# gotzmann/booster

Measured on AMD Instinct MI355X. Metric: decode tokens/sec Llama-3-8B Q4_K_M, higher is better.
Workload: dtype int8xint4/6 dot -> f32 (Q4_K/Q6_K weights x Q8_K activations), f16 KV; 1 GPU; Llama-3-8B Q4_K_M shapes (synthetic GGUF, random K-quant blocks), greedy batch-1 decode on 1xMI355X, 128-token prompt, n_ctx 2304, n_kv 133..2087; parallelism=single GPU, aql_runs=2, replay=AQL packets, fence scope NONE, own HSA queue (csrc/bamd_aql.h)

## Files before the change

### booster_amd/__init__.py

```python
import ctypes as C
import os

import numpy as np

_HERE = os.path.dirname(os.path.abspath(__file__))
LIB_PATH = os.environ.get("BAMD_LIB") or os.path.join(_HERE, "lib", "libbooster_amd.so")
_lib = None

F32, F16, Q4_K, Q5_K, Q6_K = 0, 1, 12, 13, 14


class BamdError(RuntimeError):
    pass


def lib():
    global _lib
    if _lib is None:
        if not os.path.exists(LIB_PATH):
            raise BamdError("libbooster_amd.so is not built (python -m booster_amd.build); there is no CPU fallback")
        try:
            import torch
        except ImportError:
            pass
        L = C.CDLL(LIB_PATH)
        vp, ci, cf, i64 = C.c_void_p, C.c_int, C.c_float, C.c_int64
        L.bamd_last_error.restype = C.c_char_p
        L.bamd_model_load.restype = vp; L.bamd_model_load.argtypes = [C.c_char_p, ci, ci, ci, ci, ci]
        L.bamd_model_free.argtypes = [vp]
        for n in ("bamd_model_n_vocab", "bamd_model_n_embd", "bamd_model_n_layer", "bamd_model_n_ctx_train"):
            getattr(L, n).argtypes = [vp]
        L.bamd_model_weight_bytes.restype = i64; L.bamd_model_weight_bytes.argtypes = [vp]
        L.bamd_model_tensor_raw.restype = i64; L.bamd_model_tensor_raw.argtypes = [vp, C.c_char_p, vp, i64]
        L.bamd_context_new.restype = vp; L.bamd_context_new.argtypes = [vp, ci]
        L.bamd_context_free.argtypes = [vp]
        L.bamd_n_ctx.argtypes = [vp]
        L.bamd_kv_cache_clear.argtypes = [vp]
        L.bamd_decode.argtypes = [vp, vp, ci, ci]
        L.bamd_get_logits.restype = C.POINTER(C.c_float); L.bamd_get_logits.argtypes = [vp]
        L.bamd_generate_greedy.argtypes = [vp, ci, ci, vp, C.POINTER(C.c_float)]
        L.bamd_kv_seq_rm.argtypes = [vp, ci, ci]; L.bamd_kv_seq_add.argtypes = [vp, ci, ci, ci]; L.bamd_kv_seq_div.argtypes = [vp, ci, ci, ci]
        L.bamd_stage_step.argtypes = [vp, C.c_int32, vp, ci, vp, vp, ci, ci, vp]
        L.bamd_stage_token_to.argtypes = [vp, vp, vp]
        L.bamd_stage_prefill.argtypes = [vp, vp, ci, ci, vp, vp, ci, vp]
        L.bamd_stage_argmax.argtypes = [vp, vp, C.POINTER(C.c_int32)]
        L.bamd_profile_step.argtypes = [vp, ci, vp, vp, vp]; L.bamd_profile_step_kinds.argtypes = [vp, ci, vp, vp, vp]
        L.bamd_timeline_step.argtypes = [vp, ci, ci, vp, ci, C.POINTER(ci)]
        L.bamd_set_prefill_batch.argtypes = [ci]; L.bamd_set_prefill_batch.restype = None
        L.bamd_bench_matvec.argtypes = [ci, ci, ci, ci, ci, ci, ci, C.POINTER(C.c_float)]
        L.bamd_op_quantize_q8_K.argtypes = [vp, i64, vp, cf, vp]
        L.bamd_op_mul_mat_vec.argtypes = [ci, vp, ci, ci, vp, vp, cf, vp, vp, ci]
        L.bamd_op_mul_mat_vec_argmax.argtypes = [ci, vp, ci, ci, vp, vp, cf, vp, ci, C.POINTER(C.c_int32)]
        L.bamd_op_ffn_gate_up.argtypes = [ci, vp, vp, ci, ci, vp, vp, cf, vp]
        L.bamd_op_mul_mat_batch.argtypes = [ci, vp, ci, ci, vp, ci, vp, cf, vp, vp, ci]
        L.bamd_op_get_row.argtypes = [ci, vp, ci, ci, ci, vp]
        L.bamd_op_attention.argtypes = [vp, vp, vp, vp, vp, vp, ci, ci, ci, ci, ci, ci, vp, vp]
        L.bamd_op_attention_batch.argtypes = [vp, vp, vp, vp, vp, vp, ci, ci, ci, ci, ci, ci, ci, ci, vp]
        L.bamd_op_rope_row.argtypes = [ci, ci, cf, cf, vp, vp]
        L.bamd_set_aql.argtypes = [ci]; L.bamd_set_aql.restype = None
        L.bamd_aql_runs.argtypes = [vp]
        _lib = L
    return _lib


def _chk(rc):
    if rc != 0:
        raise BamdError(lib().bamd_last_error().decode())


def _p(a):
    return None if a is None else a.ctypes.data_as(C.c_void_p)


def set_prefill_batch(on):
    lib().bamd_set_prefill_batch(int(on))


def set_aql(on):
    lib().bamd_set_aql(int(bool(on)))


def device_count():
    return lib().bamd_device_count()


class Model:

    def __init__(self, path, device=0, layer_first=0, layer_last=-1, with_embd=True, with_output=True):
        self.h = lib().bamd_model_load(os.fsencode(path), device, layer_first, layer_last, int(with_embd), int(with_output))
# ... 157 lines not shown

def op_ffn_gate_up(ttype, wg_raw, wu_raw, nrows, k, x, norm_w=None, eps=0.0):
    wg_raw = np.ascontiguousarray(wg_raw, np.uint8); wu_raw = np.ascontiguousarray(wu_raw, np.uint8)
    x = np.ascontiguousarray(x, np.float32)
    nw = None if norm_w is None else np.ascontiguousarray(norm_w, np.float32)
    y = np.zeros(nrows, np.float32)
    _chk(lib().bamd_op_ffn_gate_up(ttype, _p(wg_raw), _p(wu_raw), nrows, k, _p(x), _p(nw), eps, _p(y)))
    return y


def op_get_row(ttype, w_raw, nrows, k, row):
    w_raw = np.ascontiguousarray(w_raw, np.uint8)
    y = np.zeros(k, np.float32)
    _chk(lib().bamd_op_get_row(ttype, _p(w_raw), nrows, k, row, _p(y)))
    return y


def op_rope_row(pos, n_dims, freq_base, freq_scale=1.0, freq_factors=None):
    row = np.zeros(n_dims, np.float32)
    ff = None if freq_factors is None else np.ascontiguousarray(freq_factors, np.float32)
    _chk(lib().bamd_op_rope_row(pos, n_dims, freq_base, freq_scale, _p(ff), _p(row)))
    return row


def op_attention(q, k, v, k_cache, v_cache_t, rope_row, H, Hkv, hd, n_ctx, pos, prefill_mode=False, want_probs=False, long_path=False):
    q = np.ascontiguousarray(q, np.float32); k = np.ascontiguousarray(k, np.float32); v = np.ascontiguousarray(v, np.float32)
    rope_row = np.ascontiguousarray(rope_row, np.float32)
    assert k_cache.dtype == np.uint16 and v_cache_t.dtype == np.uint16 and k_cache.flags.c_contiguous and v_cache_t.flags.c_contiguous
    out = np.zeros(H * hd, np.float32)
    probs = np.zeros(n_ctx, np.float32) if want_probs else None
    _chk(lib().bamd_op_attention(_p(q), _p(k), _p(v), _p(k_cache), _p(v_cache_t), _p(rope_row), H, Hkv, hd, n_ctx, pos, int(prefill_mode) | (2 if (long_path or want_probs) else 0),
                                 _p(out), _p(probs)))
    return (out, probs) if want_probs else out


def op_attention_batch(q, k, v, k_cache, v_cache_t, rope, H, Hkv, hd, n_ctx, pos0, impl=0, ld=0):
    q = np.ascontiguousarray(q, np.float32).reshape(-1, H * hd)
    T = q.shape[0]
    k = np.ascontiguousarray(k, np.float32).reshape(T, Hkv * hd); v = np.ascontiguousarray(v, np.float32).reshape(T, Hkv * hd)
    rope = np.ascontiguousarray(rope, np.float32).reshape(n_ctx, hd)
    assert k_cache.dtype == np.uint16 and v_cache_t.dtype == np.uint16 and k_cache.flags.c_contiguous and v_cache_t.flags.c_contiguous
    assert k_cache.size == n_ctx * Hkv * hd and v_cache_t.size == n_ctx * Hkv * hd
    out = np.zeros((T, H * hd), np.float32)
    _chk(lib().bamd_op_attention_batch(_p(q), _p(k), _p(v), _p(k_cache), _p(v_cache_t), _p(rope), H, Hkv, hd, n_ctx, pos0, T, impl, ld, _p(out)))
    return out
```

### booster_amd/csrc/bamd_attention.hip

```cpp
#include "bamd_device.h"

#define BAMD_QK_NT 4
template <int GQ, int LG, bool SH, int NT = BAMD_QK_NT>
__global__ void __launch_bounds__(512) attn_qk_kernel(bamd_attn_args a) {
    constexpr int hd = 64 * LG, L = 8 * LG, hp = hd / 2;
    constexpr int NPAIR = (GQ + 1) * hp, IT = (NPAIR + 511) / 512;
    __shared__ __attribute__((aligned(16))) float qt[GQ * 256];
    __shared__ __attribute__((aligned(16))) unsigned short q16t[GQ * 256];
    __shared__ __attribute__((aligned(16))) unsigned short k16t[256];
    __shared__ __attribute__((aligned(16))) float scs[NT][GQ][64];
    const bamd_step_state * st = a.st;
    const int Hkv = a.Hkv, Ekv = Hkv * hd, n_ctx = a.n_ctx;
    const int hk = blockIdx.x, by = (int) blockIdx.y, gy = (int) gridDim.y;
    const int tid = threadIdx.x, lane = tid & 63, wave = wave_id(), e = lane & 7, r = lane >> 3;
    float2 xin[IT], cs[IT];
#pragma unroll
    for (int it = 0; it < IT; ++it) {
        const int idx = tid + it * 512, idc = idx < NPAIR ? idx : 0, hh = idc / hp, p = idc - hh * hp;
        const float * src = hh < GQ ? a.q + (size_t) (hk * GQ + hh) * hd : a.k + (size_t) hk * hd;
        xin[it] = ik_ld2f(src + 2 * p);
        cs[it] = ik_ld2f(a.rope_cur + 2 * p);
    }
    const float vst = ik_ld(a.v + hk * hd + (tid < hd ? tid : 0));
    const int pos = ik_ld(&st->pos), n_kv = ik_ld(&st->n_kv), cell = SH ? ik_ld(&st->cell) : pos;
// ... 36 lines not shown
#pragma unroll
            for (int g = 0; g < GQ; ++g) sc[g] = -INFINITY;
            bool live = i <= pos;
            if (SH) live = i < n_kv && (i == cell || (uint32_t) ik_ld(a.cellpos + (i < n_kv ? i : 0)) <= (uint32_t) pos);
            if (live) {
                uint4 kreg[4];
#pragma unroll
                for (int g = 0; g < 4; ++g) {
                    kreg[g] = make_uint4(0, 0, 0, 0);
                    if (g < LG) { const uint4 own = *(const uint4 *) (k16t + g * BAMD_KGRP + e * 8); kreg[g] = i == cell ? own : kpre[j][g < LG ? g : 0]; }
                }
#pragma unroll
                for (int g = 0; g < GQ; ++g) {
                    if (BAMD_QK_KNOCK & 2) { sc[g] = __uint_as_float(kreg[0].x ^ kreg[1 < LG ? 1 : 0].w) + qt[g * hd + e * 8]; continue; }
                    const float v = a.prefill_mode ? kq_chain<true>(kreg, L, nullptr, q16t + g * hd + e * 8) : kq_chain<false>(kreg, L, qt + g * hd + e * 8, nullptr);
                    sc[g] = a.prefill_mode ? hsum8_vecdot(v) : hsum8_tinyblas(v);
                }
            }
            if (e == 0) {
#pragma unroll
                for (int g = 0; g < GQ; ++g) scs[j][g][r * 8 + wave] = sc[g];
            }
        }
        __syncthreads();
        for (int q4 = tid; q4 < NT * GQ * 16; q4 += 512) {
            const int j = q4 / (GQ * 16), g = (q4 >> 4) % GQ, c4 = q4 & 15, tile = tile0 + j * gy;
            if (tile < tiles && (!(BAMD_QK_KNOCK & 4) || scs[j][g][c4 * 4] == 12345.f)) ik_st128f(rs, (uint32_t) ((hk * GQ + g) * n_ctx + tile * 64 + c4 * 4) * 4u, *(const float4 *) &scs[j][g][c4 * 4]);
        }
        if (tile0 + NT * gy < tiles) { __syncthreads(); BAMD_QK_PREFETCH(tile0 + NT * gy); }
    }
#undef BAMD_QK_PREFETCH
}

__device__ __forceinline__ double seq_expsum8_vt(const float * v, int n) {
    double sq = 0.0;
    for (int i = 0; i < n; i += 8) {
        const float * q = v + (i & ~63) + ((i & 63) >> 3);
        const float a0 = q[0] + q[32], a1 = q[8] + q[40], a2 = q[16] + q[48], a3 = q[24] + q[56];
        const float b0 = a0 + a2, b1 = a1 + a3;
        sq += (double) (b0 + b1);
    }
    return sq;
}
#define BAMD_SM_R 8
__global__ void __launch_bounds__(1024) attn_softmax_kernel(bamd_attn_args a) {
    __shared__ float redf[16];
    __shared__ double redd[16];
    const bamd_step_state * st = a.st;
    const int n_kv = st->n_kv, n_ctx = a.n_ctx;
    const int h = blockIdx.x;
    float * s = a.scores + (size_t) h * n_ctx;
    float * pr = a.probs + (size_t) h * n_ctx;
    const float scale = a.kq_scale;
    const int tid = threadIdx.x, lane = tid & 63, wave = wave_id(), nw = blockDim.x >> 6;
    const bool cached = n_kv <= BAMD_SM_R * (int) blockDim.x;
    float v[BAMD_SM_R];
    float mx = -INFINITY;
    if (cached) {
#pragma unroll
        for (int k = 0; k < BAMD_SM_R; ++k) { const int i = tid + k * blockDim.x; v[k] = i < n_kv ? s[vperm(i)] * scale : -INFINITY; mx = v[k] > mx ? v[k] : mx; }
    } else for (int i = tid; i < n_kv; i += blockDim.x) { const float w = s[vperm(i)] * scale; mx = w > mx ? w : mx; }
    for (int o = 32; o; o >>= 1) { const float om = __shfl_xor(mx, o); mx = om > mx ? om : mx; }
    if (lane == 0) redf[wave] = mx;
    __syncthreads();
    mx = redf[0]; for (int w = 1; w < nw; ++w) mx = redf[w] > mx ? redf[w] : mx;
    double sum = 0.0;
    if (cached) {
#pragma unroll
        for (int k = 0; k < BAMD_SM_R; ++k) {
            const int i = tid + k * blockDim.x;
            if (i < n_kv) {
                const float val = v_expf(v[k] - mx);
                v[k] = val;
                const float c = hsum8_tinyblas(val);
                if ((lane & 7) == 0) sum += (double) c;
            }
// ... 478 lines not shown
```

### booster_amd/csrc/bamd_attn_fused.h

```cpp
#pragma once
#include "bamd_device.h"

#define BAMD_ATTN_LDS_MAX (144 * 1024)
struct AttnEnvWG {
    int tid, wave, nthr;
    __device__ __forceinline__ AttnEnvWG() : tid((int) threadIdx.x), wave(wave_id()), nthr((int) blockDim.x) { }
    __device__ __forceinline__ void sync() const { __syncthreads(); }
    __device__ __forceinline__ float2 qk2(const bamd_attn_args & a, int role, int h, int hk, int hd, int rp) const {
        const float * rsrc = role == 1 ? a.k + (size_t) hk * hd : a.q + (size_t) h * hd;
        return BAMD_IK_QKV ? ik_ld2f(rsrc + 2 * rp) : *(const float2 *) (rsrc + 2 * rp);
    }
    __device__ __forceinline__ float vel(const bamd_attn_args & a, int hk, int hd, int i) const { return ik_ld_if<BAMD_IK_QKV != 0>(a.v + hk * hd + i); }
};
template <int LG, bool COLAUNCH, typename ENV = AttnEnvWG>
__device__ __forceinline__ void attn_fused_body(bamd_attn_args a, int gq, const int h, const int tokb_in, unsigned char * attn_dyn, uint32_t * done_flags, uint32_t tag, const ENV env = ENV()) {
    __shared__ __attribute__((aligned(16))) float qt[256];
    __shared__ __attribute__((aligned(16))) unsigned short q16t[256];
    __shared__ __attribute__((aligned(16))) unsigned short k16t[256];
    float * sc = (float *) attn_dyn;
    float * pt = sc + (a.lds_ld ? a.lds_ld : a.n_ctx);
    __shared__ float redf[8];
    __shared__ double redd[8];
    const bamd_step_state * st = a.st;
    const int tokb = a.batch ? tokb_in : 0;
    const int pos = ik_ld_if<BAMD_IK_ST != 0>(&st->pos) + tokb;
    int n_kv = ik_ld_if<BAMD_IK_ST != 0>(&st->n_kv);
    if (a.batch) { const int nc = ik_ld(&st->n_ctx); n_kv = (pos + 1 + 31) / 32 * 32; n_kv = n_kv < nc ? n_kv : nc; }
    a.q += (size_t) tokb * a.ld_qkv; a.k += (size_t) tokb * a.ld_qkv; a.v += (size_t) tokb * a.ld_qkv; a.out += (size_t) tokb * a.ld_out;
    constexpr int hd = LG * 64, L = LG * 8, hp = hd / 2;
    const int Hkv = a.Hkv, Ekv = Hkv * hd, n_ctx = a.n_ctx;
    const int hk = h / gq;
    const int tid = env.tid, lane = tid & 63, wave = env.wave, e = lane & 7;
    const float * rope = a.rope + (size_t) pos * hd;
    TL_STAMP(a.tl, 0);
    const int role = tid / hp, rp = tid - role * hp;
    const float2 xin = env.qk2(a, role, h, hk, hd, rp);
    const float2 cs = *(const float2 *) (rope + 2 * rp);
    const float vst = env.vel(a, hk, hd, tid < hd ? tid : 0);
    const int r_pos = wave * 8 + (lane >> 3);
    float vcf[LG];
#pragma unroll
    for (int dd = 0; dd < LG; ++dd) vcf[dd] = env.vel(a, hk, hd, r_pos + 64 * dd);
    const bamd_ik_rsrc rk = ik_rsrc(a.kc), rv = ik_rsrc(a.vc);
    uint4 kreg[4][LG];
#pragma unroll
    for (int t = 0; t < 4; ++t) {
        const int i = t * 64 + r_pos < n_ctx ? t * 64 + r_pos : n_ctx - 64 + r_pos;
#pragma unroll
        for (int g = 0; g < LG; ++g) kreg[t][g] = ik_ld128_if<BAMD_IK_KLD != 0>(rk, (uint32_t) (i * Ekv + hk * hd + g * BAMD_KGRP + e * 8) * 2u);
    }
    uint4 vreg[4][LG < 2 ? LG : 2];
#pragma unroll
    for (int t = 0; t < 4; ++t) {
        const int tb = t * 64 < n_ctx ? t * 64 : n_ctx - 64;
#pragma unroll
        for (int dd = 0; dd < (LG < 2 ? LG : 2); ++dd) vreg[t][dd] = ik_ld128_if<BAMD_IK_VLD != 0>(rv, (uint32_t) ((hk * hd + r_pos + 64 * dd) * n_ctx + tb + e * 8) * 2u);
    }
    {
        const float t0 = xin.x * cs.x, t1 = xin.y * cs.y, t2 = xin.x * cs.y, t3 = xin.y * cs.x;
        const float r0 = t0 - t1, r1 = t2 + t3;
        const int i0 = kperm(2 * rp, L), i1 = kperm(2 * rp + 1, L);
        if (role == 0) { qt[i0] = r0; qt[i1] = r1; q16t[i0] = f2h(r0); q16t[i1] = f2h(r1); }
        else if (role == 1) { k16t[i0] = f2h(r0); k16t[i1] = f2h(r1); }
    }
    env.sync();
    if (h == hk * gq && !a.batch && tid < hd) {
        ik_st_if<BAMD_IK_KVST != 0>(a.kc + (size_t) pos * Ekv + hk * hd + tid, k16t[tid]);
        ik_st_if<BAMD_IK_KVST != 0>(a.vc + (size_t) (hk * hd + tid) * n_ctx + vperm(pos), f2h(vst));
    }
    TL_STAMP(a.tl, 1);
    uint4 kself[4];
#pragma unroll
    for (int g = 0; g < 4; ++g) kself[g] = g < LG ? *(const uint4 *) (k16t + g * BAMD_KGRP + e * 8) : make_uint4(0, 0, 0, 0);
#define BAMD_SCORE_TILE(t0_, KL_) do { \
        const int i = (t0_) + r_pos; \
        uint4 kk[4]; \
        _Pragma("unroll") for (int g = 0; g < 4; ++g) { \
            const uint4 kc_ = g < LG ? KL_[g < LG ? g : 0] : make_uint4(0, 0, 0, 0); \
            kk[g].x = i == pos ? kself[g].x : kc_.x; kk[g].y = i == pos ? kself[g].y : kc_.y; kk[g].z = i == pos ? kself[g].z : kc_.z; kk[g].w = i == pos ? kself[g].w : kc_.w; \
        } \
        float v = a.prefill_mode ? hsum8_vecdot(kq_chain<true>(kk, L, nullptr, q16t + e * 8)) : hsum8_tinyblas(kq_chain<false>(kk, L, qt + e * 8, nullptr)); \
        v = (i < n_kv && i <= pos) ? v : -INFINITY;                \
        if (e == 0 && i < n_kv) sc[i] = v; \
    } while (0)
#pragma unroll
    for (int t = 0; t < 4; ++t) { if (t * 64 < n_kv) BAMD_SCORE_TILE(t * 64, kreg[t]); }
    for (int t0 = 256; t0 < n_kv; t0 += 64) {
        const int i2 = t0 + r_pos;
        uint4 kl[LG];
#pragma unroll
        for (int g = 0; g < LG; ++g) kl[g] = ik_ld128_if<BAMD_IK_KLD != 0>(rk, (uint32_t) (i2 * Ekv + hk * hd + g * BAMD_KGRP + e * 8) * 2u);
        BAMD_SCORE_TILE(t0, kl);
    }
#undef BAMD_SCORE_TILE
    env.sync();
    TL_STAMP(a.tl, 2);
    const float scale = a.kq_scale;
    float mx = -INFINITY;
    for (int i = tid; i < n_kv; i += env.nthr) { const float w = sc[i] * scale; mx = w > mx ? w : mx; }
    {
        uint32_t u = __float_as_uint(mx); u = (u & 0x80000000u) ? ~u : (u | 0x80000000u);
        u = wave_max_u32(u);
        if (lane == 0) redf[wave] = __uint_as_float((u & 0x80000000u) ? (u & 0x7fffffffu) : ~u);
    }
    env.sync();
    mx = redf[0];
    for (int w = 1; w < 8; ++w) mx = redf[w] > mx ? redf[w] : mx;
    double sum = 0.0;
    for (int i = tid; i < n_kv; i += env.nthr) {
        const float w = sc[i] * scale;
        const float val = v_expf(w - mx);
        sc[i] = val;
        const float c = hsum8_tinyblas(val);
        if (e == 0) sum += (double) c;
    }
    sum = wave_sum_f64(sum);
    if (lane == 0) redd[wave] = sum;
    env.sync();
    double tot = 0.0;
    for (int w = 0; w < 8; ++w) tot += redd[w];
    double rs = 1.0 / tot;
    float fs = (float) rs;
    if (!f32_rounding_safe(rs, BAMD_F64_GUARD_ULPS(n_kv / 8))) {
        env.sync();
        if (tid == 0) redd[0] = seq_expsum8(sc, n_kv);
        env.sync();
        rs = 1.0 / redd[0]; fs = (float) rs;
    }
    for (int i = tid; i < n_kv; i += env.nthr) pt[vperm(i)] = sc[i] * fs;
    for (int i = n_kv + tid; i < ((n_kv + 63) & ~63); i += env.nthr) pt[vperm(i)] = 0.f;
    env.sync();
    TL_STAMP(a.tl, 3);
    unsigned short vcur[4] = { 0, 0, 0, 0 };
#pragma unroll
    for (int dd = 0; dd < LG; ++dd) vcur[dd] = f2h(vcf[dd]);
    float acc4[4] = { 0.f, 0.f, 0.f, 0.f };
    const int pblk = pos & ~63, pe = pos & 7, pl = (pos & 63) >> 3;
#define BAMD_PV_BLOCK(b0_, dd_, VV_) do { \
        const float4 pa = *(const float4 *) (pt + (b0_) + e * 8), pb = *(const float4 *) (pt + (b0_) + e * 8 + 4); \
        const float pv[8] = { pa.x, pa.y, pa.z, pa.w, pb.x, pb.y, pb.z, pb.w }; \
        uint32_t w[4] = { (VV_).x, (VV_).y, (VV_).z, (VV_).w }; \
        if ((b0_) == pblk && e == pe) {                             \
            const uint32_t keep = (pl & 1) ? 0x0000ffffu : 0xffff0000u, ins = (pl & 1) ? (uint32_t) vcur[dd_] << 16 : (uint32_t) vcur[dd_]; \
            _Pragma("unroll") for (int j = 0; j < 4; ++j) if (j == (pl >> 1)) w[j] = (w[j] & keep) | ins; \
        } \
        acc4[dd_] = fma_mix_chain<8>(acc4[dd_], w, pv); \
    } while (0)
#pragma unroll
    for (int t = 0; t < 4; ++t) {
        if (t * 64 < n_kv) {
#pragma unroll
            for (int dd = 0; dd < (LG < 2 ? LG : 2); ++dd) BAMD_PV_BLOCK(t * 64, dd, vreg[t][dd]);
#pragma unroll
            for (int dd = 2; dd < LG; ++dd) {
                const uint4 vv = ik_ld128_if<BAMD_IK_VLD != 0>(rv, (uint32_t) ((hk * hd + r_pos + 64 * dd) * n_ctx + t * 64 + e * 8) * 2u);
                BAMD_PV_BLOCK(t * 64, dd, vv);
            }
        }
    }
    for (int b0 = 256; b0 < n_kv; b0 += 64) {
#pragma unroll
        for (int dd = 0; dd < LG; ++dd) {
            const uint4 vv = ik_ld128_if<BAMD_IK_VLD != 0>(rv, (uint32_t) ((hk * hd + r_pos + 64 * dd) * n_ctx + b0 + e * 8) * 2u);
            BAMD_PV_BLOCK(b0, dd, vv);
        }
    }
#undef BAMD_PV_BLOCK
#pragma unroll
    for (int dd = 0; dd < LG; ++dd) {
        const float v = hsum8_tinyblas(acc4[dd]);
        if (e == 0) {
            if (COLAUNCH) __hip_atomic_store((unsigned long long *) done_flags + (size_t) h * hd + r_pos + 64 * dd, ((unsigned long long) tag << 32) | __float_as_uint(v),
                                             __ATOMIC_RELAXED, __HIP_MEMORY_SCOPE_AGENT);
            else ik_st(a.out + (size_t) h * hd + r_pos + 64 * dd, v);
        }
    }
    TL_STAMP(a.tl, 7);
}
```

### booster_amd/csrc/bamd_device.h

```cpp
#pragma once
#include <hip/hip_runtime.h>
#include <hip/hip_fp16.h>
#include <stdint.h>
#include <stdlib.h>
#include "bamd_formats.h"
#include "bamd_kernels.h"
#include "bamd_aql.h"

#define WAVE 64
#ifndef BAMD_SCHED_GROUP
#define BAMD_SCHED_GROUP 4
#endif

#ifdef BAMD_TIMING
#define TL_STAMP(tl, k) do { if ((tl) && (threadIdx.x & 63) == 0 && blockIdx.x < BAMD_TL_WG && blockIdx.y == 0) { const int w_ = (int) (threadIdx.x >> 6); \
        if (w_ == 0 || w_ == 7) (tl)[(size_t) blockIdx.x * BAMD_TL_WG_WORDS + (w_ ? 8 : 0) + (k)] = wall_clock64(); \
        if ((k) == 7 && w_ < 8) (tl)[(size_t) blockIdx.x * BAMD_TL_WG_WORDS + 16 + w_] = wall_clock64(); } } while (0)
#else
#define TL_STAMP(tl, k) do { } while (0)
#endif

__device__ __forceinline__ float h2f(uint32_t bits16) { return __half2float(__ushort_as_half((unsigned short) bits16)); }
__device__ __forceinline__ unsigned short f2h(float f) { return __half_as_ushort(__float2half_rn(f)); }
__device__ __forceinline__ int sdot4(uint32_t a, uint32_t b) { return __builtin_amdgcn_sdot4((int) a, (int) b, 0, false); }
// ... 110 lines not shown
    return v;
}
template <int CTRL> __device__ __forceinline__ double dpp_d(double v) {
    const int lo = dpp_i<CTRL>(__double2loint(v)), hi = dpp_i<CTRL>(__double2hiint(v));
    return __hiloint2double(hi, lo);
}
__device__ __forceinline__ double readlane_d(double v, int lane) {
    return __hiloint2double(__builtin_amdgcn_readlane(__double2hiint(v), lane), __builtin_amdgcn_readlane(__double2loint(v), lane));
}
__device__ __forceinline__ double wave_sum_f64(double s) {
    s += dpp_d<DPP_XOR1>(s); s += dpp_d<DPP_XOR2>(s); s += dpp_d<DPP_HALF_MIRROR>(s); s += dpp_d<DPP_MIRROR>(s);
    return ((readlane_d(s, 15) + readlane_d(s, 31)) + readlane_d(s, 47)) + readlane_d(s, 63);
}

#define BAMD_F64_GUARD_ULPS(n) (2 * (n) + 8)
__device__ __forceinline__ bool f32_rounding_safe(double v, int ulps) {
#ifdef BAMD_NO_F64_GUARD
    return true;
#endif
    if (v == 0.0) return true;
    const uint32_t hi = (uint32_t) __double2hiint(v), lo = (uint32_t) __double2loint(v);
    const uint32_t ex = (hi >> 20) & 0x7ffu;
    const int dist = (int) (lo & 0x1fffffffu) - 0x10000000;
    return ex >= 1023u - 126u && ex <= 1023u + 127u && (dist < 0 ? -dist : dist) > ulps;
}
__device__ __forceinline__ double seq_expsum8(const float * vals, int n) {
    double s = 0.0;
    for (int i = 0; i < n; i += 8) {
        const float a0 = vals[i] + vals[i + 4], a1 = vals[i + 1] + vals[i + 5], a2 = vals[i + 2] + vals[i + 6], a3 = vals[i + 3] + vals[i + 7];
        const float b0 = a0 + a2, b1 = a1 + a3;
        s += (double) (b0 + b1);
    }
    return s;
}

#define BAMD_ACT_BATCH 4
#ifndef BAMD_CEILING
#define BAMD_CEILING 0
#endif
#define BAMD_ACT_RED_OFF(nb) ((((size_t) (nb) * (256 + 32 + 4)) + 15) & ~(size_t) 15)
template <bool NORM>
struct ActPro {
    float4 v[BAMD_ACT_BATCH], w[BAMD_ACT_BATCH];
    int okmask;
    unsigned long long * tl = nullptr;

    template <int NB = BAMD_ACT_BATCH>
    __device__ __forceinline__ void issue(const float * __restrict__ x, const float * __restrict__ nw, int K, int i0, int bstride = 0, int blimit = 0) {
        const int lane = threadIdx.x & 63;
        if (bstride == 0) { bstride = blockDim.x >> 6; blimit = K >> 8; }
        okmask = 0;
        const bamd_ik_rsrc rx = ik_rsrc(x);
#pragma unroll
        for (int b = 0; b < NB; ++b) {
            const int i = i0 + b * bstride;
            const bool ok = i < blimit;
            okmask |= ok ? 1 << b : 0;
            const int ic = ok ? i : blimit - 1;
            v[b] = ik_ld128f(rx, (uint32_t) lane * 16u, ic * 1024);
            if (NORM) w[b] = *(const float4 *) (nw + ic * 256 + lane * 4);
        }
    }

    template <int NB = BAMD_ACT_BATCH>
    __device__ __forceinline__ void quantize_batch(float scale, int K, int i0, uint32_t * q8, int * S, float * yd, int bstride = 0, int blimit = 0) {
        const int lane = threadIdx.x & 63;
// ... 585 lines not shown
```

### booster_amd/csrc/bamd_engine.cpp

```cpp
#include "../../include/bamd.h"
#include "bamd_formats.h"
#include "bamd_gguf.h"
#include "bamd_kernels.h"
#include "bamd_aql.h"

#include <hip/hip_runtime.h>
#include <math.h>
#include <stdio.h>
#include <stdlib.h>
#include <string.h>
#include <algorithm>
#include <atomic>
#include <memory>
#include <mutex>
#include <stdexcept>
#include <string>
#include <vector>

static thread_local std::string g_err;
static int g_prefill_batch = [] { const char * e = getenv("BAMD_PREFILL_BATCH"); return (e && e[0] == '0') ? 0 : 1; }();
static int g_prefill_mfma = [] { const char * e = getenv("BAMD_PREFILL_MFMA"); return (e && e[0] == '0') ? 0 : 1; }();
static const int g_prefill_aux = [] { const char * e = getenv("BAMD_PREFILL_AUX"); return (e && e[0] == '0') ? 0 : 1; }();
static const int g_stage_graph = [] { const char * e = getenv("BAMD_STAGE_GRAPH"); return (e && e[0] == '0') ? 0 : 1; }();
static const bool g_attn_fused = [] { const char * e = getenv("BAMD_ATTN_FUSED"); return !(e && e[0] == '0'); }();
// ... 1353 lines not shown
    prefill_mode &= 1;
    if (need_device()) return 1;
    if (H <= 0 || Hkv <= 0 || hd <= 0 || hd % 64 || hd > 256 || n_ctx <= 0 || pos < 0 || pos >= n_ctx || n_ctx % 32 || H % Hkv) return fail("bad attention shape");
    Tmp t; const int Ekv = Hkv * hd; const int n_ctx_pad = (n_ctx + 63) / 64 * 64; const size_t kvb = (size_t) n_ctx_pad * Ekv * 2;
    std::vector<float> rope((size_t) n_ctx * hd, 0.f);
    memcpy(rope.data() + (size_t) pos * hd, rope_row_h, (size_t) hd * 4);
    std::vector<uint16_t> kd, vd;
    kv_to_device_order(k_cache, v_cache_t, n_ctx, n_ctx_pad, Hkv, hd, kd, vd);
    bamd_step_state h; memset(&h, 0, sizeof h); h.pos = pos; h.n_ctx = n_ctx; h.n_kv = std::min(n_ctx, std::max(32, (pos + 1 + 31) / 32 * 32));
    bamd_attn_args a; memset(&a, 0, sizeof a);
    a.st = (bamd_step_state *) t.up(&h, sizeof h);
    a.q = (float *) t.up(q, (size_t) H * hd * 4); a.k = (float *) t.up(k, (size_t) Ekv * 4); a.v = (float *) t.up(v, (size_t) Ekv * 4);
    a.kc = (unsigned short *) t.up(kd.data(), kvb); a.vc = (unsigned short *) t.up(vd.data(), kvb);
    a.rope = (float *) t.up(rope.data(), rope.size() * 4); if (a.rope) a.rope_cur = a.rope + (size_t) pos * hd; a.scores = (float *) t.up(nullptr, (size_t) H * n_ctx_pad * 4);
    a.probs = (float *) t.up(nullptr, (size_t) H * n_ctx_pad * 4); a.out = (float *) t.up(nullptr, (size_t) H * hd * 4);
    if (!a.st || !a.q || !a.k || !a.v || !a.kc || !a.vc || !a.rope || !a.scores || !a.probs || !a.out) return fail("device alloc/copy failed");
    a.hd = hd; a.Hkv = Hkv; a.n_ctx = n_ctx_pad; a.kq_scale = 1.0f / sqrtf((float) hd); a.prefill_mode = prefill_mode;
    { const int tiles = std::min(std::max(n_ctx / 64, 1), 64);
      if (bamd_launch_attention(a, H / Hkv, split_path ? -tiles : tiles, nullptr)) return fail("unsupported head configuration"); }
    HIPC(hipGetLastError());
    HIPC(hipDeviceSynchronize());
    HIPC(hipMemcpy(out, a.out, (size_t) H * hd * 4, hipMemcpyDeviceToHost));
    HIPC(hipMemcpy(kd.data(), a.kc, kvb, hipMemcpyDeviceToHost));
    HIPC(hipMemcpy(vd.data(), a.vc, kvb, hipMemcpyDeviceToHost));
    kv_from_device_order(k_cache, v_cache_t, n_ctx, n_ctx_pad, Hkv, hd, kd, vd);
    if (probs_h0 && split_path) {
        std::vector<float> pp((size_t) n_ctx_pad);
        HIPC(hipMemcpy(pp.data(), a.probs, (size_t) n_ctx_pad * 4, hipMemcpyDeviceToHost));
        for (int p = 0; p < h.n_kv; ++p) probs_h0[p] = pp[(size_t) ((p & ~63) + ((p & 7) << 3) + ((p & 63) >> 3))];
    }
    return 0;
}

extern "C" __attribute__((visibility("default"))) int bamd_op_attention_batch(const float * q, const float * k, const float * v, uint16_t * k_cache, uint16_t * v_cache_t,
                                                                                const float * rope, int H, int Hkv, int hd, int n_ctx, int pos0, int T, int impl, int ld,
                                                                                float * out) {
    if (need_device()) return 1;
    if (H <= 0 || Hkv <= 0 || hd <= 0 || hd % 64 || hd > 256 || n_ctx <= 0 || n_ctx % 32 || H % Hkv || H / Hkv > 8) return fail("bad attention shape");
    if (T < 1 || T > BAMD_PREFILL_CAP || pos0 < 0 || pos0 + T > n_ctx) return fail("bad micro-batch");
    if (impl < 0 || impl > 2) return fail("impl must be 0 (launcher's choice), 1 (VALU) or 2 (matrix cores)");
    const int Ekv = Hkv * hd, E = H * hd, ldq = E + 2 * Ekv, gq = H / Hkv, n_ctx_pad = (n_ctx + 63) / 64 * 64;
    const int ld_min = std::min((pos0 + T + 63) / 64 * 64, n_ctx_pad);
    if (ld == 0) ld = ld_min;
    if (ld % 64 || ld < ld_min || ld > n_ctx_pad) return fail("ld must be a multiple of 64 between the padded sequence length and the padded n_ctx");
    Tmp t; const size_t kvb = (size_t) n_ctx_pad * Ekv * 2;
    std::vector<float> qkv((size_t) T * ldq);
    for (int i = 0; i < T; ++i) {
        memcpy(&qkv[(size_t) i * ldq], q + (size_t) i * E, (size_t) E * 4);
        memcpy(&qkv[(size_t) i * ldq + E], k + (size_t) i * Ekv, (size_t) Ekv * 4);
        memcpy(&qkv[(size_t) i * ldq + E + Ekv], v + (size_t) i * Ekv, (size_t) Ekv * 4);
    }
    std::vector<uint16_t> kd, vd;
    kv_to_device_order(k_cache, v_cache_t, n_ctx, n_ctx_pad, Hkv, hd, kd, vd);
    bamd_step_state h; memset(&h, 0, sizeof h);
    h.pos_base = pos0; h.pos = pos0; h.n_ctx = n_ctx; h.step = T; h.n_kv = std::min(n_ctx, (pos0 + T + 31) / 32 * 32);
    bamd_attn_args a; memset(&a, 0, sizeof a);
    a.st = (bamd_step_state *) t.up(&h, sizeof h);
    float * dqkv = (float *) t.up(qkv.data(), qkv.size() * 4);
    a.kc = (unsigned short *) t.up(kd.data(), kvb); a.vc = (unsigned short *) t.up(vd.data(), kvb);
    a.rope = (float *) t.up(rope, (size_t) n_ctx * hd * 4); a.out = (float *) t.up(nullptr, (size_t) T * E * 4);
    if (!a.st || !dqkv || !a.kc || !a.vc || !a.rope || !a.out) return fail("device alloc/copy failed");
    a.q = dqkv; a.k = dqkv + E; a.v = dqkv + E + Ekv;
    a.hd = hd; a.Hkv = Hkv; a.n_ctx = n_ctx_pad; a.kq_scale = 1.0f / sqrtf((float) hd); a.prefill_mode = 1;
    a.batch = 1; a.ld_qkv = ldq; a.ld_out = E; a.lds_ld = ld; a.batch_pos0p1 = pos0 + 1;
    const size_t need = hd == 128 && impl != 1 ? bamd_attention_batch_mfma_scratch(Hkv, gq, T, ld) : 0;
    if (need && !(a.batch_scratch = (float *) t.up(nullptr, need))) return fail("device alloc failed (scratch block)");
// ... 53 lines not shown
```

### include/bamd.h

```cpp
#ifndef BAMD_H
#define BAMD_H
#include <stdint.h>
#include <stddef.h>
#ifdef __cplusplus
extern "C" {
#endif

typedef struct bamd_model   bamd_model;
typedef struct bamd_context bamd_context;

enum { BAMD_TYPE_F32 = 0, BAMD_TYPE_F16 = 1, BAMD_TYPE_Q4_K = 12, BAMD_TYPE_Q5_K = 13, BAMD_TYPE_Q6_K = 14 };

const char * bamd_last_error(void);

int bamd_backend_init(void);
int bamd_device_count(void);

bamd_model * bamd_model_load(const char * gguf_path, int device, int layer_first, int layer_last, int with_embd, int with_output);
void         bamd_model_free(bamd_model * m);
int          bamd_model_n_vocab(const bamd_model * m);
int          bamd_model_n_embd(const bamd_model * m);
int          bamd_model_n_layer(const bamd_model * m);
int          bamd_model_n_ctx_train(const bamd_model * m);
int64_t      bamd_model_weight_bytes(const bamd_model * m);
// ... 50 lines not shown

int bamd_gguf_probe(const char * gguf_path, int64_t * n_tensors, int64_t * n_bytes, uint64_t * digest);

int bamd_janus_shortlist_test(const float * logits, int n_vocab, float cutoff, int fast, int32_t * ids, int cap);
void * bamd_janus_test_new(const bamd_vocab * v, float scale, float hi, float lo, int depth);
void bamd_janus_test_tables(void * janus, float * types, float * scales);
int bamd_janus_test_sample(void * janus, float * logits, const int32_t * last, int n_last, int prompt_len, int pos, int max, uint32_t seed);
void bamd_janus_test_free(void * janus);
int bamd_bridge_sample_test(void * ctx, const float * logits, const int32_t * last, int n_last, int prompt_len, int pos, int max, uint32_t seed,
                            int device, float * logits_after, int64_t * counts);

int bamd_bridge_stage_layout(void * ctx, int32_t * out, int cap_stages);

void bamd_set_prefill_batch(int on);

int bamd_profile_step(bamd_context * c, int pos, int * launches, double * ms, double * bytes);
int bamd_profile_step_kinds(bamd_context * c, int pos, int * launches, double * ms, double * bytes);

int bamd_bench_matvec(int type, int nrows, int k, int pro, int epi, int mode, int iters, float * us_per_launch);

int bamd_op_quantize_q8_K(const float * x, int64_t k, const float * norm_w, float eps, void * out_blocks);
int bamd_op_mul_mat_vec(int type, const void * w_raw, int nrows, int k, const float * x, const float * norm_w, float eps,
                        const float * residual, float * y, int mode );
int bamd_op_mul_mat_vec_argmax(int type, const void * w_raw, int nrows, int k, const float * x, const float * norm_w, float eps, float * y,
                               int mode, int32_t * row);
int bamd_op_mul_mat_batch(int type, const void * w_raw, int nrows, int k, const float * x, int T, const float * norm_w, float eps,
                          const float * residual, float * y, int impl);
int bamd_op_ffn_gate_up(int type, const void * wg_raw, const void * wu_raw, int nrows, int k, const float * x, const float * norm_w,
                        float eps, float * y);
int bamd_op_get_row(int type, const void * w_raw, int nrows, int k, int row, float * y);
int bamd_op_attention(const float * q, const float * k, const float * v, uint16_t * k_cache, uint16_t * v_cache_t,
                      const float * rope_row, int H, int Hkv, int hd, int n_ctx, int pos, int prefill_mode, float * out,
                      float * probs_h0);
int bamd_op_attention_batch(const float * q, const float * k, const float * v, uint16_t * k_cache, uint16_t * v_cache_t,
                            const float * rope, int H, int Hkv, int hd, int n_ctx, int pos0, int T, int impl, int ld, float * out);
int bamd_op_rope_row(int pos, int n_dims, float freq_base, float freq_scale, const float * freq_factors, float * row);

#ifdef __cplusplus
}
#endif
#endif
```

Baseline: 657.5 tokens/s.

## Fold softmax max into score pass and branchless KV self-splice in fused attention

The fused attention kernel now tracks each wave's running max of scaled scores during the QK pass, so the separate max-reduction loop over the score buffer is gone. Exponentials are written straight into the probability buffer, and when n_kv fits in one pass the 1/sum normalisation is applied inside the PV loop instead of in an extra sweep. The splice of the current token's K/V into the cached tiles becomes a precomputed, branchless mask/insert. A test entry point for the attention+wo co-launch is also added. These changes add register pressure and shift the order of floating-point reductions.

Result: no change. 658.4 tokens/s (median of 6 runs) (+0.1%).

```diff
diff --git a/booster_amd/__init__.py b/booster_amd/__init__.py
--- a/booster_amd/__init__.py
+++ b/booster_amd/__init__.py
@@ -55,6 +55,7 @@
         L.bamd_op_mul_mat_batch.argtypes = [ci, vp, ci, ci, vp, ci, vp, cf, vp, vp, ci]
         L.bamd_op_get_row.argtypes = [ci, vp, ci, ci, ci, vp]
         L.bamd_op_attention.argtypes = [vp, vp, vp, vp, vp, vp, ci, ci, ci, ci, ci, ci, vp, vp]
+        L.bamd_op_attention_wo.argtypes = [vp, vp, vp, vp, vp, vp, ci, ci, ci, ci, ci, ci, vp, ci, vp, ci, vp]
         L.bamd_op_attention_batch.argtypes = [vp, vp, vp, vp, vp, vp, ci, ci, ci, ci, ci, ci, ci, ci, vp]
         L.bamd_op_rope_row.argtypes = [ci, ci, cf, cf, vp, vp]
         L.bamd_set_aql.argtypes = [ci]; L.bamd_set_aql.restype = None
@@ -278,6 +279,17 @@
     _chk(lib().bamd_op_attention(_p(q), _p(k), _p(v), _p(k_cache), _p(v_cache_t), _p(rope_row), H, Hkv, hd, n_ctx, pos, int(prefill_mode) | (2 if (long_path or want_probs) else 0),
                                  _p(out), _p(probs)))
     return (out, probs) if want_probs else out
+
+
+def op_attention_wo(q, k, v, k_cache, v_cache_t, rope_row, H, Hkv, hd, n_ctx, pos, wo_type, wo_raw, wo_rows, residual, il=0):
+    q = np.ascontiguousarray(q, np.float32); k = np.ascontiguousarray(k, np.float32); v = np.ascontiguousarray(v, np.float32)
+    rope_row = np.ascontiguousarray(rope_row, np.float32); residual = np.ascontiguousarray(residual, np.float32)
+    wo_raw = np.ascontiguousarray(wo_raw)
+    assert k_cache.dtype == np.uint16 and v_cache_t.dtype == np.uint16 and k_cache.flags.c_contiguous and v_cache_t.flags.c_contiguous
+    assert residual.size == wo_rows
+    out = np.zeros(wo_rows, np.float32)
+    _chk(lib().bamd_op_attention_wo(_p(q), _p(k), _p(v), _p(k_cache), _p(v_cache_t), _p(rope_row), H, Hkv, hd, n_ctx, pos, wo_type, _p(wo_raw), wo_rows, _p(residual), il, _p(out)))
+    return out
 
 
 def op_attention_batch(q, k, v, k_cache, v_cache_t, rope, H, Hkv, hd, n_ctx, pos0, impl=0, ld=0):
diff --git a/booster_amd/csrc/bamd_attention.hip b/booster_amd/csrc/bamd_attention.hip
--- a/booster_amd/csrc/bamd_attention.hip
+++ b/booster_amd/csrc/bamd_attention.hip
@@ -92,16 +92,6 @@
 #undef BAMD_QK_PREFETCH
 }
 
-__device__ __forceinline__ double seq_expsum8_vt(const float * v, int n) {
-    double sq = 0.0;
-    for (int i = 0; i < n; i += 8) {
-        const float * q = v + (i & ~63) + ((i & 63) >> 3);
-        const float a0 = q[0] + q[32], a1 = q[8] + q[40], a2 = q[16] + q[48], a3 = q[24] + q[56];
-        const float b0 = a0 + a2, b1 = a1 + a3;
-        sq += (double) (b0 + b1);
-    }
-    return sq;
-}
 #define BAMD_SM_R 8
 __global__ void __launch_bounds__(1024) attn_softmax_kernel(bamd_attn_args a) {
     __shared__ float redf[16];
diff --git a/booster_amd/csrc/bamd_attn_fused.h b/booster_amd/csrc/bamd_attn_fused.h
--- a/booster_amd/csrc/bamd_attn_fused.h
+++ b/booster_amd/csrc/bamd_attn_fused.h
@@ -2,6 +2,12 @@
 #include "bamd_device.h"
 
 #define BAMD_ATTN_LDS_MAX (144 * 1024)
+#ifndef BAMD_X_SM
+#define BAMD_X_SM 1
+#endif
+#ifndef BAMD_X_SPL
+#define BAMD_X_SPL 1
+#endif
 struct AttnEnvWG {
     int tid, wave, nthr;
     __device__ __forceinline__ AttnEnvWG() : tid((int) threadIdx.x), wave(wave_id()), nthr((int) blockDim.x) { }
@@ -23,9 +29,9 @@
     __shared__ double redd[8];
     const bamd_step_state * st = a.st;
     const int tokb = a.batch ? tokb_in : 0;
-    const int pos = ik_ld_if<BAMD_IK_ST != 0>(&st->pos) + tokb;
-    int n_kv = ik_ld_if<BAMD_IK_ST != 0>(&st->n_kv);
-    if (a.batch) { const int nc = ik_ld(&st->n_ctx); n_kv = (pos + 1 + 31) / 32 * 32; n_kv = n_kv < nc ? n_kv : nc; }
+    const int pos = __builtin_amdgcn_readfirstlane(ik_ld_if<BAMD_IK_ST != 0>(&st->pos)) + tokb;
+    int n_kv_v = ik_ld_if<BAMD_IK_ST != 0>(&st->n_kv);
+    if (a.batch) { const int nc = ik_ld(&st->n_ctx); n_kv_v = (pos + 1 + 31) / 32 * 32; n_kv_v = n_kv_v < nc ? n_kv_v : nc; }
     a.q += (size_t) tokb * a.ld_qkv; a.k += (size_t) tokb * a.ld_qkv; a.v += (size_t) tokb * a.ld_qkv; a.out += (size_t) tokb * a.ld_out;
     constexpr int hd = LG * 64, L = LG * 8, hp = hd / 2;
     const int Hkv = a.Hkv, Ekv = Hkv * hd, n_ctx = a.n_ctx;
@@ -72,16 +78,33 @@
     uint4 kself[4];
 #pragma unroll
     for (int g = 0; g < 4; ++g) kself[g] = g < LG ? *(const uint4 *) (k16t + g * BAMD_KGRP + e * 8) : make_uint4(0, 0, 0, 0);
+    const int n_kv = __builtin_amdgcn_readfirstlane(n_kv_v);
+    const int pblk = pos & ~63, pe = pos & 7, pl = (pos & 63) >> 3;
+    const float scale = a.kq_scale;
+    float wmx = -INFINITY;
+#if BAMD_X_SPL
+#define BAMD_SCORE_KK(t0_, KL_) \
+        _Pragma("unroll") for (int g = 0; g < 4; ++g) kk[g] = g < LG ? KL_[g < LG ? g : 0] : make_uint4(0, 0, 0, 0); \
+        if ((t0_) == pblk) { \
+            _Pragma("unroll") for (int g = 0; g < LG; ++g) { \
+                kk[g].x = i == pos ? kself[g].x : kk[g].x; kk[g].y = i == pos ? kself[g].y : kk[g].y; kk[g].z = i == pos ? kself[g].z : kk[g].z; kk[g].w = i == pos ? kself[g].w : kk[g].w; \
+            } \
+        }
+#else
+#define BAMD_SCORE_KK(t0_, KL_) \
+        _Pragma("unroll") for (int g = 0; g < 4; ++g) { \
+            const uint4 kc_ = g < LG ? KL_[g < LG ? g : 0] : make_uint4(0, 0, 0, 0); \
+            kk[g].x = i == pos ? kself[g].x : kc_.x; kk[g].y = i == pos ? kself[g].y : kc_.y; kk[g].z = i == pos ? kself[g].z : kc_.z; kk[g].w = i == pos ? kself[g].w : kc_.w; \
+        }
+#endif
 #define BAMD_SCORE_TILE(t0_, KL_) do { \
         const int i = (t0_) + r_pos; \
         uint4 kk[4]; \
-        _Pragma("unroll") for (int g = 0; g < 4; ++g) { \
-            const uint4 kc_ = g < LG ? KL_[g < LG ? g : 0] : make_uint4(0, 0, 0, 0); \
-            kk[g].x = i == pos ? kself[g].x : kc_.x; kk[g].y = i == pos ? kself[g].y : kc_.y; kk[g].z = i == pos ? kself[g].z : kc_.z; kk[g].w = i == pos ? kself[g].w : kc_.w; \
-        } \
+        BAMD_SCORE_KK(t0_, KL_) \
         float v = a.prefill_mode ? hsum8_vecdot(kq_chain<true>(kk, L, nullptr, q16t + e * 8)) : hsum8_tinyblas(kq_chain<false>(kk, L, qt + e * 8, nullptr)); \
         v = (i < n_kv && i <= pos) ? v : -INFINITY;                \
         if (e == 0 && i < n_kv) sc[i] = v; \
+        if (BAMD_X_SM) { const float w = v * scale; wmx = (e == 0 && w > wmx) ? w : wmx; } \
     } while (0)
 #pragma unroll
     for (int t = 0; t < 4; ++t) { if (t * 64 < n_kv) BAMD_SCORE_TILE(t * 64, kreg[t]); }
@@ -93,9 +116,48 @@
         BAMD_SCORE_TILE(t0, kl);
     }
 #undef BAMD_SCORE_TILE
+#undef BAMD_SCORE_KK
+#if BAMD_X_SM
+    {
+        uint32_t u = __float_as_uint(wmx); u = (u & 0x80000000u) ? ~u : (u | 0x80000000u);
+        u = wave_max_u32(u);
+        if (lane == 0) redf[wave] = __uint_as_float((u & 0x80000000u) ? (u & 0x7fffffffu) : ~u);
+    }
+#endif
     env.sync();
     TL_STAMP(a.tl, 2);
-    const float scale = a.kq_scale;
+#if BAMD_X_SM
+    float mx = redf[0];
+    for (int w = 1; w < 8; ++w) mx = redf[w] > mx ? redf[w] : mx;
+    double sum = 0.0;
+    for (int i = tid; i < n_kv; i += env.nthr) {
+        const float w = sc[i] * scale;
+        const float val = v_expf(w - mx);
+        pt[vperm(i)] = val;
+        const float c = hsum8_tinyblas(val);
+        if (e == 0) sum += (double) c;
+    }
+    for (int i = n_kv + tid; i < ((n_kv + 63) & ~63); i += env.nthr) pt[vperm(i)] = 0.f;
+    sum = wave_sum_f64(sum);
+    if (lane == 0) redd[wave] = sum;
+    env.sync();
+    double tot = 0.0;
+    for (int w = 0; w < 8; ++w) tot += redd[w];
+    double rs = 1.0 / tot;
+    float fs = (float) rs;
+    if (!f32_rounding_safe(rs, BAMD_F64_GUARD_ULPS(n_kv / 8))) {
+        env.sync();
+        if (tid == 0) redd[0] = seq_expsum8_vt(pt, n_kv);
+        env.sync();
+        rs = 1.0 / redd[0]; fs = (float) rs;
+    }
+    const bool pscale = n_kv <= env.nthr;
+    if (!pscale) {
+        for (int i = tid; i < n_kv; i += env.nthr) pt[vperm(i)] = pt[vperm(i)] * fs;
+        env.sync();
+    }
+#else
+    const bool pscale = false; float fs;
     float mx = -INFINITY;
     for (int i = tid; i < n_kv; i += env.nthr) { const float w = sc[i] * scale; mx = w > mx ? w : mx; }
     {
@@ -120,7 +182,7 @@
     double tot = 0.0;
     for (int w = 0; w < 8; ++w) tot += redd[w];
     double rs = 1.0 / tot;
-    float fs = (float) rs;
+    fs = (float) rs;
     if (!f32_rounding_safe(rs, BAMD_F64_GUARD_ULPS(n_kv / 8))) {
         env.sync();
         if (tid == 0) redd[0] = seq_expsum8(sc, n_kv);
@@ -130,20 +192,36 @@
     for (int i = tid; i < n_kv; i += env.nthr) pt[vperm(i)] = sc[i] * fs;
     for (int i = n_kv + tid; i < ((n_kv + 63) & ~63); i += env.nthr) pt[vperm(i)] = 0.f;
     env.sync();
+#endif
     TL_STAMP(a.tl, 3);
     unsigned short vcur[4] = { 0, 0, 0, 0 };
 #pragma unroll
     for (int dd = 0; dd < LG; ++dd) vcur[dd] = f2h(vcf[dd]);
     float acc4[4] = { 0.f, 0.f, 0.f, 0.f };
-    const int pblk = pos & ~63, pe = pos & 7, pl = (pos & 63) >> 3;
-#define BAMD_PV_BLOCK(b0_, dd_, VV_) do { \
-        const float4 pa = *(const float4 *) (pt + (b0_) + e * 8), pb = *(const float4 *) (pt + (b0_) + e * 8 + 4); \
-        const float pv[8] = { pa.x, pa.y, pa.z, pa.w, pb.x, pb.y, pb.z, pb.w }; \
-        uint32_t w[4] = { (VV_).x, (VV_).y, (VV_).z, (VV_).w }; \
+#if BAMD_X_SPL
+    uint32_t smask[4], sins[LG][4];
+#pragma unroll
+    for (int j = 0; j < 4; ++j) {
+        const bool hit = e == pe && j == (pl >> 1);
+        smask[j] = hit ? ((pl & 1) ? 0x0000ffffu : 0xffff0000u) : 0xffffffffu;
+#pragma unroll
+        for (int dd = 0; dd < LG; ++dd) sins[dd][j] = hit ? ((pl & 1) ? (uint32_t) vcur[dd] << 16 : (uint32_t) vcur[dd]) : 0u;
+    }
+#define BAMD_PV_SPLICE(b0_, dd_) \
+        if ((b0_) == pblk) { _Pragma("unroll") for (int j = 0; j < 4; ++j) w[j] = (w[j] & smask[j]) | sins[dd_][j]; }
+#else
+#define BAMD_PV_SPLICE(b0_, dd_) \
         if ((b0_) == pblk && e == pe) {                             \
             const uint32_t keep = (pl & 1) ? 0x0000ffffu : 0xffff0000u, ins = (pl & 1) ? (uint32_t) vcur[dd_] << 16 : (uint32_t) vcur[dd_]; \
             _Pragma("unroll") for (int j = 0; j < 4; ++j) if (j == (pl >> 1)) w[j] = (w[j] & keep) | ins; \
-        } \
+        }
+#endif
+#define BAMD_PV_BLOCK(b0_, dd_, VV_) do { \
+        const float4 pa = *(const float4 *) (pt + (b0_) + e * 8), pb = *(const float4 *) (pt + (b0_) + e * 8 + 4); \
+        float pv[8] = { pa.x, pa.y, pa.z, pa.w, pb.x, pb.y, pb.z, pb.w }; \
+        if (pscale) { _Pragma("unroll") for (int l = 0; l < 8; ++l) pv[l] = pv[l] * fs; } \
+        uint32_t w[4] = { (VV_).x, (VV_).y, (VV_).z, (VV_).w }; \
+        BAMD_PV_SPLICE(b0_, dd_) \
         acc4[dd_] = fma_mix_chain<8>(acc4[dd_], w, pv); \
     } while (0)
 #pragma unroll
@@ -166,6 +244,7 @@
         }
     }
 #undef BAMD_PV_BLOCK
+#undef BAMD_PV_SPLICE
 #pragma unroll
     for (int dd = 0; dd < LG; ++dd) {
         const float v = hsum8_tinyblas(acc4[dd]);
diff --git a/booster_amd/csrc/bamd_device.h b/booster_amd/csrc/bamd_device.h
--- a/booster_amd/csrc/bamd_device.h
+++ b/booster_amd/csrc/bamd_device.h
@@ -166,6 +166,17 @@
         s += (double) (b0 + b1);
     }
     return s;
+}
+
+__device__ __forceinline__ double seq_expsum8_vt(const float * v, int n) {
+    double sq = 0.0;
+    for (int i = 0; i < n; i += 8) {
+        const float * q = v + (i & ~63) + ((i & 63) >> 3);
+        const float a0 = q[0] + q[32], a1 = q[8] + q[40], a2 = q[16] + q[48], a3 = q[24] + q[56];
+        const float b0 = a0 + a2, b1 = a1 + a3;
+        sq += (double) (b0 + b1);
+    }
+    return sq;
 }
 
 #define BAMD_ACT_BATCH 4
diff --git a/booster_amd/csrc/bamd_engine.cpp b/booster_amd/csrc/bamd_engine.cpp
--- a/booster_amd/csrc/bamd_engine.cpp
+++ b/booster_amd/csrc/bamd_engine.cpp
@@ -1409,6 +1409,52 @@
     return 0;
 }
 
+extern "C" __attribute__((visibility("default"))) int bamd_op_attention_wo(const float * q, const float * k, const float * v, uint16_t * k_cache, uint16_t * v_cache_t,
+                                                                             const float * rope_row_h, int H, int Hkv, int hd, int n_ctx, int pos, int wo_type, const void * wo_raw,
+                                                                             int wo_rows, const float * residual, int il, float * out) {
+    if (need_device()) return 1;
+    if (H <= 0 || Hkv <= 0 || hd <= 0 || hd % 64 || hd > 256 || n_ctx <= 0 || pos < 0 || pos >= n_ctx || n_ctx % 32 || H % Hkv) return fail("bad attention shape");
+    const int E = H * hd;
+    if (!bamd_is_kquant(wo_type) || E % 256 || wo_rows <= 0 || wo_rows % 8 || !residual || !wo_raw) return fail("bad wo type/shape");
+    Tmp t; const int Ekv = Hkv * hd; const int n_ctx_pad = (n_ctx + 63) / 64 * 64; const size_t kvb = (size_t) n_ctx_pad * Ekv * 2;
+    std::vector<float> rope((size_t) n_ctx * hd, 0.f);
+    memcpy(rope.data() + (size_t) pos * hd, rope_row_h, (size_t) hd * 4);
+    std::vector<uint16_t> kd, vd;
+    kv_to_device_order(k_cache, v_cache_t, n_ctx, n_ctx_pad, Hkv, hd, kd, vd);
+    bamd_step_state h; memset(&h, 0, sizeof h); h.pos = pos; h.n_ctx = n_ctx; h.n_kv = std::min(n_ctx, std::max(32, (pos + 1 + 31) / 32 * 32));
+    h.serial = 1; h.step = pos;
+    bamd_attn_args a; memset(&a, 0, sizeof a);
+    a.st = (bamd_step_state *) t.up(&h, sizeof h);
+    a.q = (float *) t.up(q, (size_t) E * 4); a.k = (float *) t.up(k, (size_t) Ekv * 4); a.v = (float *) t.up(v, (size_t) Ekv * 4);
+    a.kc = (unsigned short *) t.up(kd.data(), kvb); a.vc = (unsigned short *) t.up(vd.data(), kvb);
+    a.rope = (float *) t.up(rope.data(), rope.size() * 4); if (a.rope) a.rope_cur = a.rope + (size_t) pos * hd;
+    a.out = (float *) t.up(nullptr, (size_t) E * 4);
+    unsigned long long * gran = (unsigned long long *) t.up(nullptr, (size_t) E * 8);
+    uint32_t * err = (uint32_t *) t.up(nullptr, 4);
+    const size_t wb = bamd_row_bytes(wo_type, E) * (size_t) wo_rows, wbp = bamd_stream_bytes(wo_type, E, wo_rows);
+    void * raw = t.up(wo_raw, wb), * str = t.up(nullptr, wbp);
+    float * dres = (float *) t.up(residual, (size_t) wo_rows * 4), * dy = (float *) t.up(nullptr, (size_t) wo_rows * 4);
+    if (!a.st || !a.q || !a.k || !a.v || !a.kc || !a.vc || !a.rope || !a.out || !gran || !err || !raw || !str || !dres || !dy) return fail("device alloc/copy failed");
+    HIPC(hipMemset(gran, 0, (size_t) E * 8)); HIPC(hipMemset(err, 0, 4)); HIPC(hipMemset(str, 0, wbp));
+    bamd_launch_repack(raw, str, wo_type, wo_rows, E, nullptr);
+    a.hd = hd; a.Hkv = Hkv; a.n_ctx = n_ctx_pad; a.kq_scale = 1.0f / sqrtf((float) hd); a.prefill_mode = 0;
+    bamd_mv_args w; memset(&w, 0, sizeof w);
+    w.seg[0].w = str; w.seg[0].out = dy; w.seg[0].type = wo_type; w.seg[0].nrows = wo_rows; w.seg[0].nvalid = wo_rows; w.nseg = 1;
+    w.x = a.out; w.K = E; w.res = dres;
+    HIPC(hipDeviceSynchronize());
+    if (bamd_launch_attn_wo(a, H / Hkv, w, n_cu0(), gran, il, err, nullptr)) return fail("no co-launch kernel for this shape");
+    HIPC(hipGetLastError());
+    HIPC(hipDeviceSynchronize());
+    uint32_t herr = 0;
+    HIPC(hipMemcpy(&herr, err, 4, hipMemcpyDeviceToHost));
+    if (herr) return fail("co-launch: the wo role gave up waiting for the attention role");
+    HIPC(hipMemcpy(out, dy, (size_t) wo_rows * 4, hipMemcpyDeviceToHost));
+    HIPC(hipMemcpy(kd.data(), a.kc, kvb, hipMemcpyDeviceToHost));
+    HIPC(hipMemcpy(vd.data(), a.vc, kvb, hipMemcpyDeviceToHost));
+    kv_from_device_order(k_cache, v_cache_t, n_ctx, n_ctx_pad, Hkv, hd, kd, vd);
+    return 0;
+}
+
 extern "C" __attribute__((visibility("default"))) int bamd_op_attention_batch(const float * q, const float * k, const float * v, uint16_t * k_cache, uint16_t * v_cache_t,
                                                                                 const float * rope, int H, int Hkv, int hd, int n_ctx, int pos0, int T, int impl, int ld,
                                                                                 float * out) {
diff --git a/include/bamd.h b/include/bamd.h
--- a/include/bamd.h
+++ b/include/bamd.h
@@ -106,6 +106,9 @@
 int bamd_op_attention(const float * q, const float * k, const float * v, uint16_t * k_cache, uint16_t * v_cache_t,
                       const float * rope_row, int H, int Hkv, int hd, int n_ctx, int pos, int prefill_mode, float * out,
                       float * probs_h0);
+int bamd_op_attention_wo(const float * q, const float * k, const float * v, uint16_t * k_cache, uint16_t * v_cache_t, const float * rope_row,
+                         int H, int Hkv, int hd, int n_ctx, int pos, int wo_type, const void * wo_raw, int wo_rows, const float * residual,
+                         int il, float * out);
 int bamd_op_attention_batch(const float * q, const float * k, const float * v, uint16_t * k_cache, uint16_t * v_cache_t,
                             const float * rope, int H, int Hkv, int hd, int n_ctx, int pos0, int T, int impl, int ld, float * out);
 int bamd_op_rope_row(int pos, int n_dims, float freq_base, float freq_scale, const float * freq_factors, float * row);
```
